# junghoseong/aircombat-selfplay

Hardware: AMD Instinct MI355X
Metric: agent-steps/sec (higher is better)
Workload: dtype f32

## Files before the change

aircombat-selfplay_amd/csrc/aircombat.hip:

```cpp
#include <hip/hip_runtime.h>
#include <stdint.h>
#include <stdio.h>
#include <string.h>
#include <string>
#include <vector>
#include <cmath>
#include <algorithm>
#include <chrono>
#include "../../include/aircombat.h"
#include "../../include/aircombat_buffer.h"
#include "clk_stamps.hpp"
#include "f16_device.hpp"
#include "f16_split.hpp"

using f16::State;
using f16::Derived;
using f16::Tab;
using f16::clampf;

#define AC_F_FIELDS(X)                                                                                           \
  X(vx) X(vy) X(vz) X(q0) X(q1) X(q2) X(q3) X(wp) X(wq) X(wr) X(hv1x) X(hv1y) X(hv1z) X(hv2x) X(hv2y) X(hv2z)   \
  X(ha1x) X(ha1y) X(ha1z) X(wdx) X(wdy) X(wdz) X(aix) X(aiy) X(aiz) X(bax) X(bay) X(baz) X(da) X(de) X(dr)       \
  X(thr) X(pin_r) X(pin_p) X(pin_y) X(pi_r) X(pi_p) X(pi_y) X(tef) X(ail) X(elev) X(sbdeg) X(alpha) X(mach)      \
  X(qc) X(vg) X(ap) X(aq) X(ar) X(npx) X(npy) X(npz) X(n1) X(n2) X(n2norm) X(ff) X(tank0) X(tank1)
// ... 156 lines not shown
    s.npz = v.x; s.npx = v.y; s.eng = __float_as_int(v.z); s.ticks = __float_as_int(v.w);
  }
  if (ROLE != 1) load_position(D, N, n, s);
}
__device__ __forceinline__ void load_flight(const float* F, const int* I, const double* D, int N, int n, State& s) { load_flight_role<-1>(F, I, D, N, n, s); }
__device__ __forceinline__ void store_flight(float* F, int* I, double* D, int N, int n, const State& s) {
  (void)I;
  AC_LANE_INDEX(n);
#define G(g, a, b, c, d) AC_GRP(F, g) = make_float4(s.a, s.b, s.c, s.d);
  AC_FLIGHT_GROUPS(G)
#undef G
  AC_GRP(F, 6) = make_float4(s.npz, s.npx, __int_as_float(s.eng), __int_as_float(s.ticks));
  store_position(D, N, n, s);
}
__device__ __forceinline__ void load_task(const float* F, const int* I, int N, int n, Task& t) {
  (void)I;
  AC_LANE_INDEX(n);
  const float4 a = AC_GRP(F, SG_TASK0), b = AC_GRP(F, SG_TASK0 + 1), c = AC_GRP(F, SG_TASK0 + 2), d = AC_GRP(F, SG_TASK0 + 3);
  t.pre_posture = a.x; t.pre_altitude = a.y; t.pre_event = a.z; t.cur_step = __float_as_int(a.w);
  t.bloods = b.x; t.status = __float_as_int(b.y); t.die_flag = __float_as_int(b.z); t.pre_shoot = b.w;
  t.remaining = __float_as_int(c.x); t.pre_remaining = __float_as_int(c.y); t.shoot_action = __float_as_int(c.z); t.last_missile = __float_as_int(c.w);
  t.last_shoot_time = __float_as_int(d.x); t.lock_bits = __float_as_int(d.y); t.lock_pos = __float_as_int(d.z);
}
__device__ __forceinline__ void store_task_group0(float* F, int N, int n, const Task& t) {
  AC_LANE_INDEX(n);
  AC_GRP(F, SG_TASK0) = make_float4(t.pre_posture, t.pre_altitude, t.pre_event, __int_as_float(t.cur_step));
}
__device__ __forceinline__ void store_task_rare(float* F, int N, int n, const Task& t) {
  AC_LANE_INDEX(n);
  AC_GRP(F, SG_TASK0 + 1) = make_float4(t.bloods, __int_as_float(t.status), __int_as_float(t.die_flag), t.pre_shoot);
  AC_GRP(F, SG_TASK0 + 2) = make_float4(__int_as_float(t.remaining), __int_as_float(t.pre_remaining), __int_as_float(t.shoot_action), __int_as_float(t.last_missile));
  AC_GRP(F, SG_TASK0 + 3) = make_float4(__int_as_float(t.last_shoot_time), __int_as_float(t.lock_bits), __int_as_float(t.lock_pos), 0.0f);
}
__device__ __forceinline__ void store_task(float* F, int* I, int N, int n, const Task& t) {
  (void)I;
  store_task_group0(F, N, n, t);
  store_task_rare(F, N, n, t);
}
__device__ __forceinline__ void load_state(const float* F, const int* I, const double* D, int N, int n, State& s, Task& t) {
  load_flight(F, I, D, N, n, s);
  load_task(F, I, N, n, t);
}
__device__ __forceinline__ void store_state(float* F, int* I, double* D, int N, int n, const State& s, const Task& t) {
  store_flight(F, I, D, N, n, s);
  store_task(F, I, N, n, t);
}
// ... 51 lines not shown
  float n, e, u;
  double n64, e64, u64;
  float vn, ve, vd;
  float alt_m;
  float ub, vb, wb, vc;
  float sphi, cphi, stht, ctht;
  float m11, m12;
};
__device__ __forceinline__ float mps(float fps) { return clampf(-700.0f, fps * f16::kFt2M, 700.0f); }

__device__ __forceinline__ void make_pose(const Derived& d, const DevCfg& c, Props& p) {
  p.alt_m = clampf(-500.0f, d.h_sl_ft * f16::kFt2M, 26000.0f);
  p.vn = mps(d.vn); p.ve = mps(d.ve); p.vd = mps(d.vd);
  const double a = 6378137.0, b = 6356752.314245179;
  double sl = d.sLat64, cl = d.cLat64, so = d.sLon64, co = d.cLon64;
  double Nn = a * a * fx::rsqrt(a * a * cl * cl + b * b * sl * sl);
  double h = (double)p.alt_m;
  double x = (Nn + h) * cl * co, y = (Nn + h) * cl * so, z = (Nn * (b / a) * (b / a) + h) * sl;
  double dx = x - c.P0x, dy = y - c.P0y, dz = z - c.P0z;
  double t = c.cLon0 * dx + c.sLon0 * dy;
  p.e64 = -c.sLon0 * dx + c.cLon0 * dy; p.u64 = c.cLat0 * t + c.sLat0 * dz; p.n64 = -c.sLat0 * t + c.cLat0 * dz;
  p.e = (float)p.e64; p.u = (float)p.u64; p.n = (float)p.n64;
}
__device__ __forceinline__ void make_props(const State& s, const Derived& d, const DevCfg& c, Props& p) {
  make_pose(d, c, p);
  p.ub = mps(d.u); p.vb = mps(d.v); p.wb = mps(d.w);
  p.vc = clampf(0.0f, f16::vcas_from_impact_pressure(s.qc) * f16::kFt2M, 1400.0f);
  const float* T = d.T;
  float m13 = T[0] * d.d_eci[0] + T[1] * d.d_eci[1] + T[2] * d.d_eci[2];
  float m23 = T[3] * d.d_eci[0] + T[4] * d.d_eci[1] + T[5] * d.d_eci[2];
  float m33 = T[6] * d.d_eci[0] + T[7] * d.d_eci[1] + T[8] * d.d_eci[2];
  p.m11 = T[0] * d.n_eci[0] + T[1] * d.n_eci[1] + T[2] * d.n_eci[2];
  p.m12 = T[0] * d.e_eci[0] + T[1] * d.e_eci[1] + T[2] * d.e_eci[2];
  p.stht = clampf(-1.0f, -m13, 1.0f);
  float ct = sqrtf(fmaxf(0.0f, 1.0f - p.stht * p.stht));
  p.ctht = ct;
  float ic = (ct > 1e-12f) ? 1.0f / sqrtf(m23 * m23 + m33 * m33) : 0.0f;
  p.sphi = (ct > 1e-12f) ? m23 * ic : 0.0f;
  p.cphi = (ct > 1e-12f) ? m33 * ic : 1.0f;
}

struct Geo { float AO, TA, R, side, cAO, cTA; };
__device__ __forceinline__ float acos_fast(float x) { return f16::atan2_fast(sqrtf((1.0f - x) * (1.0f + x)), x); }
__device__ __forceinline__ float tanh_fast(float x) {
  const float t = __expf(2.0f * clampf(-10.0f, x, 10.0f));
  return (t - 1.0f) / (t + 1.0f);
}
__device__ __forceinline__ float atanh_fast(float x) { return 0.5f * __logf((1.0f + x) / (1.0f - x)); }
template <bool TWO_D>
__device__ __forceinline__ Geo ao_ta_r(float ex, float ey, float ez, float evx, float evy, float evz,
                                       float nx, float ny, float nz, float nvx, float nvy, float nvz) {
  float dx = nx - ex, dy = ny - ey, dz = nz - ez;
  float ev, nv, R, pe, pn;
  if (TWO_D) {
    ev = sqrtf(evx * evx + evy * evy); nv = sqrtf(nvx * nvx + nvy * nvy); R = sqrtf(dx * dx + dy * dy);
    pe = dx * evx + dy * evy; pn = dx * nvx + dy * nvy;
  } else {
    ev = sqrtf(evx * evx + evy * evy + evz * evz); nv = sqrtf(nvx * nvx + nvy * nvy + nvz * nvz);
    R = sqrtf(dx * dx + dy * dy + dz * dz);
    pe = dx * evx + dy * evy + dz * evz; pn = dx * nvx + dy * nvy + dz * nvz;
  }
  Geo g;
// ... 388 lines not shown
  PairLds& LP = QUAD ? LQ.P : *reinterpret_cast<PairLds*>(split_lds);
  const Tab T{lds_tab};
  const int N = c.N;
  const int l = threadIdx.x & 63;
  const int n = blockIdx.x * 64 + l;
  const bool live = n < N;
  const int nn = live ? n : (N - 2 + (n & 1));
  const int slot = nn & 1;

  State s; Task t; Derived d; Props pr;
  int pre_st[MSLOTS];
#pragma unroll
  for (int k = 0; k < MSLOTS; ++k) pre_st[k] = MSL_INACTIVE;
  const float* act = P.actions + (size_t)nn * c.act_dim;
  float4 a4;
  ActionFetch arow;
  float shoot_raw = 0.0f;
  if (SPLIT) {
    TableCopy<192> tc;
    tc.issue(P.tab);
    AC_CLKW(0, 123);
    const int role = __builtin_amdgcn_readfirstlane(threadIdx.x >> 6);
    s = State{}; t = Task{};
    if (role == 0) { load_flight_role<0>(P.F, P.I, P.D, N, nn, s); AC_CLKW(0, 124); load_task(P.F, P.I, N, nn, t); AC_CLKW(0, 125); }
    else if (role == 1) load_flight_role<1>(P.F, P.I, P.D, N, nn, s);
    else { load_flight_role<2>(P.F, P.I, P.D, N, nn, s); t.status = state_word(P.F, SW_status, N, nn); }
    __builtin_amdgcn_s_barrier();
    tc.write(lds_tab);
    a4 = make_float4(0.f, 0.f, 0.f, 0.f);
    __builtin_amdgcn_s_waitcnt(0x0F70);
    if (role == 1) arow.issue(act, c.act_dim);
    AC_CLKW(0, 120); AC_CLKW(1, 121); AC_CLKW(2, 122);
    __syncthreads();
  } else if (QUAD) {
    const int role = __builtin_amdgcn_readfirstlane(threadIdx.x >> 6);
    TableCopy<256> tc;
    tc.issue(P.tab);
    s = State{}; t = Task{};
    if (role == 0) { load_flight_role<0>(P.F, P.I, P.D, N, nn, s); t.status = state_word(P.F, SW_status, N, nn); }
    else if (role == 1) load_flight_role<1>(P.F, P.I, P.D, N, nn, s);
    else if (role == 2) { load_flight_role<2>(P.F, P.I, P.D, N, nn, s); t.status = state_word(P.F, SW_status, N, nn); }
    else {
      load_task(P.F, P.I, N, nn, t);
      s.ticks = state_word(P.F, SW_ticks, N, nn);
#pragma unroll
      for (int k = 0; k < MSLOTS; ++k) pre_st[k] = P.MI[((size_t)k * NMI + MI_status) * (size_t)N + nn];
    }
    __builtin_amdgcn_s_barrier();
    tc.write(lds_tab);
// ... 10 lines not shown
      a4 = make_float4(0.f, 0.f, 0.f, 0.f);
      s = State{}; load_task(P.F, P.I, N, nn, t);
#pragma unroll
      for (int k = 0; k < MSLOTS; ++k) pre_st[k] = P.MI[((size_t)k * NMI + MI_status) * (size_t)N + nn];
    }
    stage_tables<128>(lds_tab, P.tab);
    if (flight_role) {
      pair_flight_load(P, c, nn, fin);
      pair_flight_wave<true>(P, c, T, LP, l, n, live, fin);
      return;
    }

  } else {
    TableCopy<64> tc;
    tc.issue(P.tab);
    a4 = load_controls(act, c.act_dim);
    if (TASK == AC_TASK_SHOOT_MISSILE) shoot_raw = act[4];
    load_state(P.F, P.I, P.D, N, nn, s, t);
    tc.commit(lds_tab);
  }
  AC_CLK(1);
  const Task was = t;
  constexpr bool OBS_BY_KIN = SPLIT && TASK == AC_TASK_SINGLECOMBAT;
  if (SPLIT) {
    const int role = __builtin_amdgcn_readfirstlane(threadIdx.x >> 6);
    if (split_helper_wave(s, t, T, L, l, c.substeps, nullptr, nullptr, &arow)) {
      if (OBS_BY_KIN && role == 1) {
        using namespace mail;
        wg_sync();
        Props q;
        q.alt_m = L.M[T_PR][l]; q.ub = L.M[T_PR + 5][l];
        q.n = L.M[T_PR + 9][l]; q.e = L.M[T_PR + 10][l]; q.u = L.M[T_PR + 11][l];
        q.vn = L.M[T_PR + 12][l]; q.ve = L.M[T_PR + 13][l]; q.vd = L.M[T_PR + 14][l];
        const Enemy Eq = exchange_1v1(q);
        L.M[T_RALT][l] = altitude_raw(q, c);
        L.M[T_RPOS][l] = posture_raw(q, Eq);
        wg_sync();
      }
      if (OBS_BY_KIN && role == 2) {
        using namespace mail;
        wg_sync();
        Props q;
        q.alt_m = L.M[T_PR][l]; q.sphi = L.M[T_PR + 1][l]; q.cphi = L.M[T_PR + 2][l]; q.stht = L.M[T_PR + 3][l]; q.ctht = L.M[T_PR + 4][l];
        q.ub = L.M[T_PR + 5][l]; q.vb = L.M[T_PR + 6][l]; q.wb = L.M[T_PR + 7][l]; q.vc = L.M[T_PR + 8][l];
        q.n = L.M[T_PR + 9][l]; q.e = L.M[T_PR + 10][l]; q.u = L.M[T_PR + 11][l];
        q.vn = L.M[T_PR + 12][l]; q.ve = L.M[T_PR + 13][l]; q.vd = L.M[T_PR + 14][l];
        const Enemy Eq = exchange_1v1(q);
        const Incoming none{false, 0, 0, 0, 0, 0, 0};
        float obq[OBS];
        observe_1v1<TASK>(q, Eq, none, obq);
        wg_sync();
        if (L.M[T_DONE][l] != 0.0f) {
          const float* tobs = (const float*)(P.tF + (size_t)NSW * 2) + slot * OBS;
#pragma unroll
          for (int k = 0; k < OBS; ++k) obq[k] = tobs[k];
        }
        float* row = lds_out + l * OBS;
#pragma unroll
        for (int k = 0; k < OBS; ++k) row[k] = obq[k];
        emit_obs_rows(P, lds_out, OBS, l);
      }
      return;
    }
  }
  Msl ms[MSLOTS];
  int nslots = 0, msl_was_active = 0;
  if (HAS_MSL) {
    nslots = min(c.num_missiles[slot], MSLOTS);
#pragma unroll
    for (int k = 0; k < MSLOTS; ++k) {
      const int st = (k < nslots) ? (PAIR ? pre_st[k] : P.MI[((size_t)k * NMI + MI_status) * (size_t)N + nn]) : MSL_INACTIVE;
      if (st != MSL_INACTIVE) { load_msl(P.MF, P.MI, N, nn, k, ms[k]); msl_was_active |= 1 << k; }
      else { ms[k] = Msl{}; ms[k].status = MSL_INACTIVE; }
    }
  }

  t.cur_step += 1;
  if (!SPLIT) {
    s.da = clampf(-1.0f, a4.x / 20.0f - 1.0f, 1.0f);
    s.de = clampf(-1.0f, a4.y / 20.0f - 1.0f, 1.0f);
    s.dr = clampf(-1.0f, a4.z / 20.0f - 1.0f, 1.0f);
    s.thr = clampf(0.0f, a4.w / 58.0f + 0.4f, 0.9f);
  }
  if (TASK == AC_TASK_SHOOT_MISSILE && !PAIR) t.shoot_action = (shoot_raw != 0.0f) ? 1 : 0;

  const MslParam MP = aim9l();
  bool have_pose = false;
  int last_tick = -1;
  bool env_has_missiles = false;
  if (PAIR) {
    bool mine = false;
#pragma unroll
    for (int k = 0; k < MSLOTS; ++k) mine = mine || ms[k].status != MSL_INACTIVE;
    const int other = __shfl_xor((int)mine, 1);
    env_has_missiles = mine || (bool)other;
  }
  int quad_nrun = 0;
  const int quad_ticks0 = s.ticks;
  for (int sub = 0; sub < c.substeps; ++sub) {
    bool fly_munitions = HAS_MSL;
    if (QUAD) {
      quad_substep_begin<true>(t, LQ, l, sub, env_has_missiles, quad_ticks0, quad_nrun, pr, c);
      fly_munitions = env_has_missiles;
    } else if (PAIR) {
      AC_CLK(2 + 8 * sub);
      pair_substep<true>(t, LP, l, sub, env_has_missiles, pr, c);
      AC_CLK(4 + 8 * sub);
      if (!env_has_missiles) continue;
    } else if (SPLIT) {
      if (dynamics_wave_tick(s, t, d, T, L, l, sub)) { have_pose = true; last_tick = sub; }
    } else if (t.status == AC_ALIVE) {
      if (t.bloods <= 0.0f) t.status = AC_SHOTDOWN;
      f16::tick<false>(s, d, T);
      have_pose = true;
    }
    if (HAS_MSL && fly_munitions) {
      if (!PAIR) {
      f16::locate(s, d);
      if (!have_pose) { f16::body_frame(s, d); have_pose = true; }
      make_props(s, d, c, pr);
      }
      float tx = __shfl_xor(pr.n, 1), ty = __shfl_xor(pr.e, 1), tz = __shfl_xor(pr.u, 1);
      float tvx = __shfl_xor(pr.vn, 1), tvy = __shfl_xor(pr.ve, 1), tvz = __shfl_xor(pr.vd, 1);
      bool talive = __shfl_xor(t.status, 1) == AC_ALIVE;
      bool hit_now = false;
#pragma unroll
      for (int k = 0; k < MSLOTS; ++k) {
        if (k < nslots && ms[k].status != MSL_INACTIVE) {
          missile_run(ms[k], MP, tx, ty, tz, tvx, tvy, tvz, talive, c);
          if (ms[k].status == MSL_HIT && talive) { hit_now = true; talive = false; }
        }
      }
      if (__shfl_xor((int)hit_now, 1) && t.status == AC_ALIVE) t.status = AC_SHOTDOWN;
      AC_CLK(5 + 8 * sub);
    }
    if (QUAD) wg_sync();
  }
  const bool split_located = SPLIT && dynamics_wave_finish(s, d, L, l, last_tick, c.substeps);
  if (PAIR) {
    if (QUAD) wg_sync();
    wg_sync();
    pair_read_final(LP, l, s, d, pr);
  } else if (!HAS_MSL || c.substeps == 0) {
    if (!split_located) f16::locate(s, d);
    if (!have_pose) f16::body_frame(s, d);
    make_props(s, d, c, pr);
  }
  AC_CLK(52);
  if (OBS_BY_KIN) {
    using namespace mail;
    L.M[T_PR][l] = pr.alt_m; L.M[T_PR + 1][l] = pr.sphi; L.M[T_PR + 2][l] = pr.cphi; L.M[T_PR + 3][l] = pr.stht; L.M[T_PR + 4][l] = pr.ctht;
    L.M[T_PR + 5][l] = pr.ub; L.M[T_PR + 6][l] = pr.vb; L.M[T_PR + 7][l] = pr.wb; L.M[T_PR + 8][l] = pr.vc;
    L.M[T_PR + 9][l] = pr.n; L.M[T_PR + 10][l] = pr.e; L.M[T_PR + 11][l] = pr.u;
    L.M[T_PR + 12][l] = pr.vn; L.M[T_PR + 13][l] = pr.ve; L.M[T_PR + 14][l] = pr.vd;
    wg_sync();
  }
  Enemy E = exchange_1v1(pr);

  if (c.use_artillery) {
    Geo g = ao_ta_r<false>(pr.n, pr.e, pr.u, pr.vn, pr.ve, pr.vd, E.n, E.e, E.u, E.vn, E.ve, E.vd);
    bool ealive = __shfl_xor(t.status, 1) == AC_ALIVE;
    float of = (g.AO <= 0.5236f) ? 1.0f - g.AO / 0.5236f : 0.0f;
    float Rk = g.R * 0.001f;
    float df = (Rk <= 1.0f) ? 1.0f : ((Rk <= 3.0f) ? (3.0f - Rk) * 0.5f : 0.0f);
    float dmg = ealive ? of * df : 0.0f;
    t.bloods -= __shfl_xor(dmg, 1);
  }
  if (HAS_MSL) {
    bool launch;
    if (TASK == AC_TASK_SHOOT_MISSILE && PAIR) t.shoot_action = ((QUAD ? LQ.S.M[mail::F_BITS][l] : LP.FIN[pair::FIN_BITS][l]) != 0.0f) ? 1 : 0;
    if (TASK == AC_TASK_DODGE_MISSILE) {
      const float dx = E.n - pr.n, dy = E.e - pr.e, dz = E.u - pr.u;
      const float dist = sqrtf(dx * dx + dy * dy + dz * dz);
      const float sp = sqrtf(pr.vn * pr.vn + pr.ve * pr.ve + pr.vd * pr.vd);
      const float ang = 57.29577951f * acosf(clampf(-1.0f, (dx * pr.vn + dy * pr.ve + dz * pr.vd) / (dist * sp + 1e-8f), 1.0f));
      const int len = c.lock_len;
      const unsigned bit = 1u << (unsigned)(t.lock_pos % len);
      t.lock_bits = (ang < c.max_attack_angle) ? (t.lock_bits | (int)bit) : (t.lock_bits & ~(int)bit);
      t.lock_pos += 1;
// ... 24 lines not shown
      t.remaining -= 1;
    }
  }

  Incoming inc{false, 0, 0, 0, 0, 0, 0};
  int my_hits = 0;
  int inc_slot = -1;
  if (HAS_MSL) {
    int best = 0x7fffffff, mine = -1;
#pragma unroll
    for (int k = 0; k < MSLOTS; ++k) {
      if (k < nslots && ms[k].status == MSL_LAUNCHED && ms[k].order < best) { best = ms[k].order; mine = k; }
      if (k < nslots && ms[k].status == MSL_HIT) my_hits += 1;
    }
    float a0 = 0, a1 = 0, a2 = 0, a3 = 0, a4 = 0, a5 = 0;
#pragma unroll
    for (int k = 0; k < MSLOTS; ++k)
      if (k == mine) { a0 = ms[k].px; a1 = ms[k].py; a2 = ms[k].pz; a3 = ms[k].vx; a4 = ms[k].vy; a5 = ms[k].vz; }
    inc.any = __shfl_xor((int)(mine >= 0), 1);
    inc_slot = __shfl_xor(mine, 1);
    inc.px = __shfl_xor(a0, 1); inc.py = __shfl_xor(a1, 1); inc.pz = __shfl_xor(a2, 1);
    inc.vx = __shfl_xor(a3, 1); inc.vy = __shfl_xor(a4, 1); inc.vz = __shfl_xor(a5, 1);
  }
  float ob[OBS];
  if (!OBS_BY_KIN) observe_1v1<TASK>(pr, E, inc, ob);
  AC_CLK(58);

  const int status_pre = t.status;
  int code = AC_DONE_NONE;
  bool done = false;
  bool nonfinite = false;
  {
    float np_max = fmaxf(fabsf(s.npx), fmaxf(fabsf(s.npy), fabsf(s.npz)));
    float pqr = sqrtf(d.p * d.p + d.q * d.q + d.r * d.r);
    nonfinite = nonfinite_probe(d.veci, pqr, d.h_sl_ft, np_max);
    bool extreme = nonfinite || (d.veci >= 1e10f) || (pqr >= 1000.0f) || (d.h_sl_ft >= 1e10f) || (np_max > 10.0f);
    bool overload = (s.ticks >= kTickOverload) &&
                    (fabsf(s.npx) > c.acc_x || fabsf(s.npy) > c.acc_y || fabsf(s.npz + 1.0f) > c.acc_z);
    if (pr.alt_m <= c.altitude_limit) { t.status = AC_CRASH; code = AC_DONE_LOW_ALTITUDE; done = true; }
    else if (extreme) { t.status = AC_CRASH; code = AC_DONE_EXTREME_STATE; done = true; }
    else if (overload) { t.status = AC_CRASH; code = AC_DONE_OVERLOAD; done = true; }
  }
  {
    int other_pre = __shfl_xor(status_pre, 1), other_post = __shfl_xor(t.status, 1);
    int enemy_status = (slot == 0) ? other_pre : other_post;
    if (!done) {
      if (t.status == AC_SHOTDOWN) { code = AC_DONE_SHOTDOWN; done = true; }
      else if (t.status == AC_CRASH) { code = AC_DONE_CRASHED; done = true; }
      else if (enemy_status != AC_ALIVE && !inc.any) { code = AC_DONE_MISSION_COMPLETE; done = true; }
      else if (t.cur_step >= c.max_steps) { code = AC_DONE_TIMEOUT; done = true; }
    }
  }

  const int other_done = __shfl_xor((int)done, 1);
  const bool all_done = done && (bool)other_done;
  const int other_code = __shfl_xor(code, 1);
  if (OBS_BY_KIN) {
    L.M[mail::T_DONE][l] = all_done ? 1.0f : 0.0f;
    wg_sync();
  } else if (all_done) {
    const float* tobs = (const float*)(P.tF + (size_t)NSW * 2) + slot * OBS;
#pragma unroll
    for (int k = 0; k < OBS; ++k) ob[k] = tobs[k];
  }

  AC_CLK(59);
  float reward = 0.0f;
  const bool evaluates = !t.die_flag;
  if (evaluates) {
    t.die_flag = (t.status != AC_ALIVE) ? 1 : 0;
    float r_alt = potential(OBS_BY_KIN ? L.M[mail::T_RALT][l] : altitude_raw(pr, c), c.altitude_scale, c.altitude_pot, t.pre_altitude);
    float r_pos = potential(OBS_BY_KIN ? L.M[mail::T_RPOS][l] : posture_raw(pr, E), c.posture_scale, c.posture_pot, t.pre_posture);
    float ev = ((t.status != AC_ALIVE) ? -200.0f : 0.0f) + 200.0f * (float)my_hits;
    float r_ev = potential(ev, c.event_scale, c.event_pot, t.pre_event);
    reward = r_alt + r_pos + r_ev;
    if (TASK == AC_TASK_SHOOT_MISSILE) {
      float sp = (t.remaining == t.pre_remaining - 1) ? -30.0f : 0.0f;
      t.pre_remaining = t.remaining;
      reward += potential(sp, c.shoot_penalty_scale, c.shoot_pot, t.pre_shoot);
    }
  }
  if (TASK == AC_TASK_DODGE_MISSILE) {
    float spd[MSLOTS];
#pragma unroll
    for (int k = 0; k < MSLOTS; ++k) spd[k] = sqrtf(ms[k].vx * ms[k].vx + ms[k].vy * ms[k].vy + ms[k].vz * ms[k].vz);
    const int base = (threadIdx.x & 63) - slot;
    const int my_inc_id = inc.any ? 1 + (slot ^ 1) * MSLOTS + inc_slot : 0;
    int prev = t.shoot_action;
    float r_mp = 0.0f;
#pragma unroll
    for (int i = 0; i < 2; ++i) {
      const int ev_i = __shfl((int)evaluates, base + i), id_i = __shfl(my_inc_id, base + i);
      if (!ev_i) continue;
      if (id_i) {
        if (!prev) prev = id_i;
        float v_prev = 0.0f, v_cur = 0.0f;
#pragma unroll
        for (int k = 0; k < MSLOTS; ++k) {
          float a = __shfl(spd[k], base + (prev - 1) / MSLOTS), b = __shfl(spd[k], base + (id_i - 1) / MSLOTS);
          if (k == (prev - 1) % MSLOTS) v_prev = a;
          if (k == (id_i - 1) % MSLOTS) v_cur = b;
        }
        if (slot == i) {
          const float v_dec = (v_prev - v_cur) / 340.0f * c.missile_posture_scale;
          const float va = sqrtf(pr.vn * pr.vn + pr.ve * pr.ve + pr.vd * pr.vd);
          const float ang = (inc.vx * pr.vn + inc.vy * pr.ve + inc.vz * pr.vd) / (v_cur * va);
          r_mp = (ang < 0.0f) ? ang / (fmaxf(v_dec, 0.0f) + 1.0f) : ang * fmaxf(v_dec, 0.0f);
        }
      } else prev = 0;
    }
    t.shoot_action = prev;
    reward += r_mp;
  }

  int step_out = t.cur_step;
  if (all_done) {
    load_state(P.tF, P.tI, P.tD, 2, slot, s, t);
    zero_controller_state(P, N, n, live);
#pragma unroll
    for (int k = 0; k < MSLOTS; ++k) { ms[k] = Msl{}; ms[k].status = MSL_INACTIVE; }
  }
  AC_CLK(53);
  if (live) {
    if (!PAIR) { store_flight(P.F, P.I, P.D, N, n, s); store_task_changed(P.F, P.I, N, n, t, was); }
    else {
      if (all_done) store_flight(P.F, P.I, P.D, N, n, s);
      store_task_changed(P.F, P.I, N, n, t, was);
    }
    if (HAS_MSL) {
#pragma unroll
      for (int k = 0; k < MSLOTS; ++k)
        if (k < nslots && (ms[k].status != MSL_INACTIVE || ((msl_was_active >> k) & 1))) store_msl(P.MF, P.MI, N, n, k, ms[k]);
    }
  }
  AC_CLK(55);
  reward = poison_if(nonfinite, reward);
  if (OBS_BY_KIN) emit_scalars(P, l, reward, done, 2, step_out, other_code ? other_code : code, 0, all_done ? 1 : 0);
  else emit_outputs(P, lds_out, OBS, l, ob, reward, done, 2, step_out, other_code ? other_code : code, 0, all_done ? 1 : 0);
  AC_CLK(54);
}

__device__ __forceinline__ Enemy gather_pose(const Props& pr, int lane) {
  Enemy E;
  E.n = __shfl(pr.n, lane); E.e = __shfl(pr.e, lane); E.u = __shfl(pr.u, lane);
  E.vn = __shfl(pr.vn, lane); E.ve = __shfl(pr.ve, lane); E.vd = __shfl(pr.vd, lane);
  E.ub = __shfl(pr.ub, lane); E.alt = __shfl(pr.alt_m, lane);
  return E;
}
template <int A>
__device__ __forceinline__ float observe_nvn(const Props& pr, int slot, int base_lane, int n_ego, float* ob) {
  auto c10 = [](float v) { return clampf(-10.0f, v, 10.0f); };
  if (ob) {
    ob[0] = c10(pr.alt_m / 5000.0f);
    ob[1] = c10(pr.sphi); ob[2] = c10(pr.cphi); ob[3] = c10(pr.stht); ob[4] = c10(pr.ctht);
    ob[5] = c10(pr.ub / 340.0f); ob[6] = c10(pr.vb / 340.0f); ob[7] = c10(pr.wb / 340.0f); ob[8] = c10(pr.vc / 340.0f);
  }
  const int my_team = slot < n_ego ? 0 : 1;
  const int n_mine = my_team == 0 ? n_ego : A - n_ego;
  float posture = 0.0f;
#pragma unroll
  for (int j = 0; j < A; ++j) {
// ... 1382 lines not shown
```

aircombat-selfplay_amd/csrc/split_kernel.hpp:

```cpp
#pragma once

namespace mail {
enum { RUNF,
       CTH, VB,
       MACH, QBAR, RHO, TEMP, HSL, ALPHA, BETA, QC, VG, NPY, NPZ, AP, AQ, AR,
       S_AIL, S_FLAP, S_ELEV, S_RUD, S_LEF, S_SB,
       THRUST,
       LK_CLB, LK_CNB, LK_G7,
       MASS0 = LK_G7 + 4, MASS_N = 18,
       F_TEF = MASS0 + MASS_N, F_PINR, F_PINP, F_PINY, F_PIR, F_PIP, F_PIY, F_AIL, F_ELEV, F_SBDEG, F_N1, F_N2, F_N2NORM, F_FF, F_TANK0, F_TANK1,
       F_ENG, F_DA, F_DE, F_DR, F_THR,
       F_BITS,
       K_W, K_V = K_W + 3,
       K_OUT = K_V + 3, K_OUT_N = 27,
       G_Q = K_OUT + K_OUT_N,
       G_H = G_Q + 8, G_NED = G_H + 1,
       QP_F = G_NED + 8, QP_F_N = 9,
       T_PR = QP_F + 2 * QP_F_N, T_PR_N = 15,
       T_DONE = T_PR + T_PR_N,
       T_RALT = T_DONE + 1, T_RPOS,
       ROWS = T_RPOS + 1 };
enum { GD_R, GD_X = GD_R + 6, GD_LAT = GD_X + 3, GD_QP = GD_LAT + 4, DROWS = GD_QP + 6 };
}
__device__ __forceinline__ void post_kin(float (*M)[64], int l, const f16::KinOut& o) {
  const float v[mail::K_OUT_N] = {o.T[0], o.T[1], o.T[2], o.T[3], o.T[4], o.T[5], o.T[6], o.T[7], o.T[8], o.h_sl_ft, o.n_eci[0], o.n_eci[1], o.n_eci[2],
                                  o.e_eci[0], o.e_eci[1], o.d_eci[0], o.d_eci[1], o.d_eci[2], o.gx, o.gy, o.gz, o.rxf, o.ryf, o.A.T, o.A.P, o.A.rho, o.A.a};
#pragma unroll
  for (int i = 0; i < mail::K_OUT_N; ++i) M[mail::K_OUT + i][l] = v[i];
}
__device__ __forceinline__ void fetch_kin(float (*M)[64], int l, f16::KinOut& o) {
  float v[mail::K_OUT_N];
#pragma unroll
  for (int i = 0; i < mail::K_OUT_N; ++i) v[i] = M[mail::K_OUT + i][l];
#pragma unroll
  for (int i = 0; i < 9; ++i) o.T[i] = v[i];
  o.h_sl_ft = v[9]; o.n_eci[0] = v[10]; o.n_eci[1] = v[11]; o.n_eci[2] = v[12]; o.e_eci[0] = v[13]; o.e_eci[1] = v[14];
  o.d_eci[0] = v[15]; o.d_eci[1] = v[16]; o.d_eci[2] = v[17]; o.gx = v[18]; o.gy = v[19]; o.gz = v[20]; o.rxf = v[21]; o.ryf = v[22];
  o.A.T = v[23]; o.A.P = v[24]; o.A.rho = v[25]; o.A.a = v[26];
}
__device__ __forceinline__ void post_mass(float (*M)[64], int l, const f16::DynVars& k) {
  const float v[mail::MASS_N] = {k.mass, k.cgx, k.cgy, k.cgz, k.Jxx, k.Jyy, k.Jzz, k.Jxy, k.Jxz, k.Jyz, k.c00, k.c01, k.c02, k.c11, k.c12, k.c22, k.idet, k.im_};
#pragma unroll
  for (int i = 0; i < mail::MASS_N; ++i) M[mail::MASS0 + i][l] = v[i];
}
// ... 152 lines not shown
      MD[GD_LAT][l] = d.sLat64; MD[GD_LAT + 1][l] = d.cLat64; MD[GD_LAT + 2][l] = d.sLon64; MD[GD_LAT + 3][l] = d.cLon64;
    }
    AC_CLKW(2, 69 + sub * 8);
    wg_sync();
    if (run) {
      f16::DynVars kl{};
      f16::Derived dd{};
      dd.h_sl_ft = 1e6f;
      kl.alpha = M[ALPHA][l]; kl.beta = M[BETA][l]; kl.mach = M[MACH][l]; kl.vt = 1.0f;
      f16::dyn_p3(dd, T, kl, f16::Surf{});
      M[LK_CLB][l] = kl.clb; M[LK_CNB][l] = kl.cnb;
      M[LK_G7][l] = kl.g7.x; M[LK_G7 + 1][l] = kl.g7.y; M[LK_G7 + 2][l] = kl.g7.z; M[LK_G7 + 3][l] = kl.g7.w;
    }
    if (run && !last) {
      f16::kin_attitude(s, o);
      post_kin(M, l, o);
    }
    AC_CLKW(2, 70 + sub * 8);
    wg_sync();
    if (POSE && run && !last) post_quad_pose(M, MD, l, (sub + 1) & 1, s, ticks0 + sub + 2, *cfg);
  }
  wg_sync();
}
struct SplitLds {
  float M[mail::ROWS][64];
  double MD[mail::DROWS][64];
};
template <bool QUAD = false, bool POSE = false>
__device__ __forceinline__ bool split_helper_wave(f16::State& s, Task& t, const f16::Tab& T, SplitLds& L, int l, int substeps, const float4* raw = nullptr,
                                                  const DevCfg* cfg = nullptr, ActionFetch* row = nullptr) {
  const int role = __builtin_amdgcn_readfirstlane(threadIdx.x >> 6);
  if (role == 2) { kinematics_wave<QUAD, POSE>(s, t, T, L.M, L.MD, l, substeps, cfg); return true; }
  if (role == 1) { systems_wave(s, t, T, L.M, l, substeps, raw, row); return true; }
  return false;
}
template <bool QUAD = false>
__device__ __forceinline__ bool dynamics_wave_tick(f16::State& s, Task& t, f16::Derived& d, const f16::Tab& T, SplitLds& L, int l, int sub, bool* d_stale = nullptr) {
  using namespace mail;
  float (*M)[64] = L.M;
  double (*MD)[64] = L.MD;
  bool run = t.status == AC_ALIVE;
  if (!QUAD && run && t.bloods <= 0.0f) t.status = AC_SHOTDOWN;
  f16::DynVars k;
  AC_CLK(2 + sub * 8);
  if (!QUAD) M[RUNF][l] = run ? 1.0f : 0.0f;
  const float b_wp = s.wp, b_wq = s.wq, b_wr = s.wr, b_vx = s.vx, b_vy = s.vy, b_vz = s.vz, b_ax = s.ha1x, b_ay = s.ha1y, b_az = s.ha1z;
  const float b_h1x = s.hv1x, b_h1y = s.hv1y, b_h1z = s.hv1z, b_h2x = s.hv2x, b_h2y = s.hv2y, b_h2z = s.hv2z;
  const int b_ticks = s.ticks;
  if (QUAD && !run) { M[K_V][l] = s.vx; M[K_V + 1][l] = s.vy; M[K_V + 2][l] = s.vz; }
  if (run) {
    if (sub == 0) f16::dyn_p1(s, d, k);
    else {
      f16::KinOut o;
      fetch_kin(M, l, o);
      f16::dyn_p1_lite(s, d, k, o);
    }
    M[K_W][l] = s.wp; M[K_W + 1][l] = s.wq; M[K_W + 2][l] = s.wr;
    M[K_V][l] = s.vx; M[K_V + 1][l] = s.vy; M[K_V + 2][l] = s.vz;
    M[CTH][l] = d.T[6] * d.d_eci[0] + d.T[7] * d.d_eci[1] + d.T[8] * d.d_eci[2];
    M[VB][l] = d.v;
  }
  AC_CLK(3 + sub * 8);
  wg_sync();
  AC_CLK(4 + sub * 8);
  if (QUAD && run && M[RUNF][l] == 0.0f) {
    s.wp = b_wp; s.wq = b_wq; s.wr = b_wr; s.vx = b_vx; s.vy = b_vy; s.vz = b_vz; s.ha1x = b_ax; s.ha1y = b_ay; s.ha1z = b_az; s.ticks = b_ticks;
    s.hv1x = b_h1x; s.hv1y = b_h1y; s.hv1z = b_h1z; s.hv2x = b_h2x; s.hv2y = b_h2y; s.hv2z = b_h2z;
    t.status = AC_SHOTDOWN;
    run = false;
    if (d_stale) *d_stale = true;
  }
  if (run) {
    fetch_mass(M, l, k);
    if (sub == 0) f16::dyn_p2<false>(s, d, k);
    else f16::dyn_p2<true>(s, d, k);
    M[BETA][l] = k.beta;
    M[MACH][l] = k.mach; M[QBAR][l] = k.qbar; M[RHO][l] = k.A.rho; M[TEMP][l] = k.A.T; M[HSL][l] = d.h_sl_ft;
    M[ALPHA][l] = k.alpha; M[QC][l] = k.qc; M[VG][l] = k.vg; M[NPY][l] = k.npy; M[NPZ][l] = k.npz;
    M[AP][l] = d.p; M[AQ][l] = d.q; M[AR][l] = d.r;
  }
  AC_CLK(5 + sub * 8);
  wg_sync();
  AC_CLK(6 + sub * 8);
  f16::Surf sf{};
  if (run) {
    sf = f16::Surf{M[S_AIL][l], M[S_FLAP][l], M[S_ELEV][l], M[S_RUD][l], M[S_LEF][l], M[S_SB][l], 0.0f};
    f16::dyn_p3(d, T, k, sf);
  }
  AC_CLK(7 + sub * 8);
  wg_sync();
  AC_CLK(8 + sub * 8);
  if (run) {
    k.clb = M[LK_CLB][l]; k.cnb = M[LK_CNB][l];
    k.g7 = make_float4(M[LK_G7][l], M[LK_G7 + 1][l], M[LK_G7 + 2][l], M[LK_G7 + 3][l]);
    f16::dyn_p4(s, d, k, sf, M[THRUST][l]);
    if (sub > 0) {
      const int pb = sub & 1;
      s.rx = MD[GD_R + 3 * pb][l]; s.ry = MD[GD_R + 3 * pb + 1][l]; s.rz = MD[GD_R + 3 * pb + 2][l];
    }
  }
  return run;
}
__device__ __forceinline__ bool dynamics_wave_finish(f16::State& s, f16::Derived& d, SplitLds& L, int l, int last_tick, int substeps) {
  using namespace mail;
  float (*M)[64] = L.M;
  double (*MD)[64] = L.MD;
  AC_CLK(50);
  wg_sync();
  AC_CLK(51);
  s.tef = M[F_TEF][l]; s.pin_r = M[F_PINR][l]; s.pin_p = M[F_PINP][l]; s.pin_y = M[F_PINY][l];
  s.pi_r = M[F_PIR][l]; s.pi_p = M[F_PIP][l]; s.pi_y = M[F_PIY][l]; s.ail = M[F_AIL][l]; s.elev = M[F_ELEV][l]; s.sbdeg = M[F_SBDEG][l];
  s.n1 = M[F_N1][l]; s.n2 = M[F_N2][l]; s.n2norm = M[F_N2NORM][l]; s.ff = M[F_FF][l]; s.tank0 = M[F_TANK0][l]; s.tank1 = M[F_TANK1][l];
  s.eng = __float_as_int(M[F_ENG][l]);
  s.da = M[F_DA][l]; s.de = M[F_DE][l]; s.dr = M[F_DR][l]; s.thr = M[F_THR][l];
  if (last_tick >= 1) {
    const int pb = last_tick & 1;
    s.q0 = M[G_Q + 4 * pb][l]; s.q1 = M[G_Q + 4 * pb + 1][l]; s.q2 = M[G_Q + 4 * pb + 2][l]; s.q3 = M[G_Q + 4 * pb + 3][l];
  }
  if (last_tick < 0 || last_tick != substeps - 1) return false;
  d.X = MD[GD_X][l]; d.Y = MD[GD_X + 1][l]; d.Z = MD[GD_X + 2][l];
  d.sLat64 = MD[GD_LAT][l]; d.cLat64 = MD[GD_LAT + 1][l]; d.sLon64 = MD[GD_LAT + 2][l]; d.cLon64 = MD[GD_LAT + 3][l];
  d.h_sl_ft = M[G_H][l];
  d.n_eci[0] = M[G_NED][l]; d.n_eci[1] = M[G_NED + 1][l]; d.n_eci[2] = M[G_NED + 2][l];
  d.e_eci[0] = M[G_NED + 3][l]; d.e_eci[1] = M[G_NED + 4][l]; d.e_eci[2] = 0.0f;
  d.d_eci[0] = M[G_NED + 5][l]; d.d_eci[1] = M[G_NED + 6][l]; d.d_eci[2] = M[G_NED + 7][l];
  return true;
}
__device__ __forceinline__ bool dynamics_wave_ticks(f16::State& s, Task& t, f16::Derived& d, const f16::Tab& T, SplitLds& L, int l, int substeps,
                                                    int& nrun) {
  int last_tick = -1;
  nrun = 0;
  for (int sub = 0; sub < substeps; ++sub)
    if (dynamics_wave_tick(s, t, d, T, L, l, sub)) { last_tick = sub; nrun += 1; }
  const bool located = dynamics_wave_finish(s, d, L, l, last_tick, substeps);
  if (last_tick >= 0 && !located) { f16::locate(s, d); return true; }
  return located;
}
```

Measured before the change: 234.0 million.

## Move env/reward/obs work onto kinematics wave in split kernel

Restructures the three-wave SingleCombat kernel: the kinematics wave now runs the environment step itself (locate, pose, observation, reward, task stores), the dynamics wave only flies and stores flight state, and the systems wave only emits observation rows. Before, pose props were staged through LDS and observation/reward raw values were computed redundantly on helper waves with extra barriers. Dynamics now publishes body-frame data to new mailbox rows on the last tick, so kinematics can build props without recomputing. This rebalances work across waves and removes the LDS prop round-trip, at the cost of more complex cross-wave synchronisation and a higher chance of ordering bugs.

```diff
diff --git a/aircombat-selfplay_amd/csrc/aircombat.hip b/aircombat-selfplay_amd/csrc/aircombat.hip
--- a/aircombat-selfplay_amd/csrc/aircombat.hip
+++ b/aircombat-selfplay_amd/csrc/aircombat.hip
@@ -202,6 +202,11 @@
   t.remaining = __float_as_int(c.x); t.pre_remaining = __float_as_int(c.y); t.shoot_action = __float_as_int(c.z); t.last_missile = __float_as_int(c.w);
   t.last_shoot_time = __float_as_int(d.x); t.lock_bits = __float_as_int(d.y); t.lock_pos = __float_as_int(d.z);
 }
+__device__ __forceinline__ void load_task_status(const float* F, int N, int n, Task& t) {
+  AC_LANE_INDEX(n);
+  const float4 b = AC_GRP(F, SG_TASK0 + 1);
+  t.bloods = b.x; t.status = __float_as_int(b.y);
+}
 __device__ __forceinline__ void store_task_group0(float* F, int N, int n, const Task& t) {
   AC_LANE_INDEX(n);
   AC_GRP(F, SG_TASK0) = make_float4(t.pre_posture, t.pre_altitude, t.pre_event, __int_as_float(t.cur_step));
@@ -299,8 +304,7 @@
   p.e64 = -c.sLon0 * dx + c.cLon0 * dy; p.u64 = c.cLat0 * t + c.sLat0 * dz; p.n64 = -c.sLat0 * t + c.cLat0 * dz;
   p.e = (float)p.e64; p.u = (float)p.u64; p.n = (float)p.n64;
 }
-__device__ __forceinline__ void make_props(const State& s, const Derived& d, const DevCfg& c, Props& p) {
-  make_pose(d, c, p);
+__device__ __forceinline__ void make_body_props(const State& s, const Derived& d, Props& p) {
   p.ub = mps(d.u); p.vb = mps(d.v); p.wb = mps(d.w);
   p.vc = clampf(0.0f, f16::vcas_from_impact_pressure(s.qc) * f16::kFt2M, 1400.0f);
   const float* T = d.T;
@@ -315,6 +319,10 @@
   float ic = (ct > 1e-12f) ? 1.0f / sqrtf(m23 * m23 + m33 * m33) : 0.0f;
   p.sphi = (ct > 1e-12f) ? m23 * ic : 0.0f;
   p.cphi = (ct > 1e-12f) ? m33 * ic : 1.0f;
+}
+__device__ __forceinline__ void make_props(const State& s, const Derived& d, const DevCfg& c, Props& p) {
+  make_pose(d, c, p);
+  make_body_props(s, d, p);
 }
 
 struct Geo { float AO, TA, R, side, cAO, cTA; };
@@ -749,9 +757,12 @@
     AC_CLKW(0, 123);
     const int role = __builtin_amdgcn_readfirstlane(threadIdx.x >> 6);
     s = State{}; t = Task{};
-    if (role == 0) { load_flight_role<0>(P.F, P.I, P.D, N, nn, s); AC_CLKW(0, 124); load_task(P.F, P.I, N, nn, t); AC_CLKW(0, 125); }
+    if (role == 0) { load_flight_role<0>(P.F, P.I, P.D, N, nn, s); AC_CLKW(0, 124); load_task_status(P.F, N, nn, t); AC_CLKW(0, 125); }
     else if (role == 1) load_flight_role<1>(P.F, P.I, P.D, N, nn, s);
-    else { load_flight_role<2>(P.F, P.I, P.D, N, nn, s); t.status = state_word(P.F, SW_status, N, nn); }
+    else {
+      load_flight_role<2>(P.F, P.I, P.D, N, nn, s); load_task(P.F, P.I, N, nn, t);
+      s.qc = __int_as_float(state_word(P.F, SW_qc, N, nn)); s.npy = __int_as_float(state_word(P.F, SW_npy, N, nn));
+    }
     __builtin_amdgcn_s_barrier();
     tc.write(lds_tab);
     a4 = make_float4(0.f, 0.f, 0.f, 0.f);
@@ -808,46 +819,44 @@
   AC_CLK(1);
   const Task was = t;
   constexpr bool OBS_BY_KIN = SPLIT && TASK == AC_TASK_SINGLECOMBAT;
+  static_assert(OBS_BY_KIN == SPLIT, "the three-wave form of this kernel is SingleCombat's");
   if (SPLIT) {
+    using namespace mail;
     const int role = __builtin_amdgcn_readfirstlane(threadIdx.x >> 6);
-    if (split_helper_wave(s, t, T, L, l, c.substeps, nullptr, nullptr, &arow)) {
-      if (OBS_BY_KIN && role == 1) {
-        using namespace mail;
-        wg_sync();
-        Props q;
-        q.alt_m = L.M[T_PR][l]; q.ub = L.M[T_PR + 5][l];
-        q.n = L.M[T_PR + 9][l]; q.e = L.M[T_PR + 10][l]; q.u = L.M[T_PR + 11][l];
-        q.vn = L.M[T_PR + 12][l]; q.ve = L.M[T_PR + 13][l]; q.vd = L.M[T_PR + 14][l];
-        const Enemy Eq = exchange_1v1(q);
-        L.M[T_RALT][l] = altitude_raw(q, c);
-        L.M[T_RPOS][l] = posture_raw(q, Eq);
-        wg_sync();
+    if (role == 1) {
+      systems_wave(s, t, T, L.M, l, c.substeps, nullptr, &arow);
+      AC_CLKW(1, 203);
+      emit_obs_rows(P, lds_out, OBS, l);
+      AC_CLKW(1, 206);
+      return;
+    }
+    if (role == 0) {
+      int last_tick = -1;
+      for (int sub = 0; sub < c.substeps; ++sub)
+        if (dynamics_wave_tick<false, true>(s, t, d, T, L, l, sub, nullptr, sub + 1 == c.substeps)) last_tick = sub;
+      dynamics_wave_finish<false>(s, d, L, l, last_tick, c.substeps);
+      AC_CLK(53);
+      if (L.M[T_DONE][l] != 0.0f) {
+        load_flight(P.tF, P.tI, P.tD, 2, slot, s);
+        zero_controller_state(P, N, n, live);
       }
-      if (OBS_BY_KIN && role == 2) {
-        using namespace mail;
-        wg_sync();
-        Props q;
-        q.alt_m = L.M[T_PR][l]; q.sphi = L.M[T_PR + 1][l]; q.cphi = L.M[T_PR + 2][l]; q.stht = L.M[T_PR + 3][l]; q.ctht = L.M[T_PR + 4][l];
-        q.ub = L.M[T_PR + 5][l]; q.vb = L.M[T_PR + 6][l]; q.wb = L.M[T_PR + 7][l]; q.vc = L.M[T_PR + 8][l];
-        q.n = L.M[T_PR + 9][l]; q.e = L.M[T_PR + 10][l]; q.u = L.M[T_PR + 11][l];
-        q.vn = L.M[T_PR + 12][l]; q.ve = L.M[T_PR + 13][l]; q.vd = L.M[T_PR + 14][l];
-        const Enemy Eq = exchange_1v1(q);
-        const Incoming none{false, 0, 0, 0, 0, 0, 0};
-        float obq[OBS];
-        observe_1v1<TASK>(q, Eq, none, obq);
-        wg_sync();
-        if (L.M[T_DONE][l] != 0.0f) {
-          const float* tobs = (const float*)(P.tF + (size_t)NSW * 2) + slot * OBS;
-#pragma unroll
-          for (int k = 0; k < OBS; ++k) obq[k] = tobs[k];
-        }
-        float* row = lds_out + l * OBS;
-#pragma unroll
-        for (int k = 0; k < OBS; ++k) row[k] = obq[k];
-        emit_obs_rows(P, lds_out, OBS, l);
-      }
+      if (live) store_flight(P.F, P.I, P.D, N, n, s);
+      AC_CLK(55);
       return;
     }
+    const int lt = kinematics_wave_env(s, t, T, L.M, L.MD, l, c.substeps, c, d, pr);
+    AC_CLKW(2, 200);
+    if (lt >= 0) {
+#pragma unroll
+      for (int i = 0; i < E_T_N; ++i) d.T[i] = L.M[E_T + i][l];
+      d.u = L.M[E_U][l]; d.v = L.M[VB][l]; d.w = L.M[E_W][l];
+      d.p = L.M[AP][l]; d.q = L.M[AQ][l]; d.r = L.M[AR][l];
+      d.vn = L.M[E_VN][l]; d.ve = L.M[E_VE][l]; d.vd = L.M[E_VD][l]; d.veci = L.M[E_VECI][l];
+      s.qc = L.M[QC][l]; s.npx = L.M[E_NPX][l]; s.npy = L.M[NPY][l]; s.npz = L.M[NPZ][l];
+      t.status = __float_as_int(L.M[E_STATUS][l]);
+    } else f16::body_frame(s, d);
+    pr.vn = mps(d.vn); pr.ve = mps(d.ve); pr.vd = mps(d.vd);
+    make_body_props(s, d, pr);
   }
   Msl ms[MSLOTS];
   int nslots = 0, msl_was_active = 0;
@@ -872,7 +881,6 @@
 
   const MslParam MP = aim9l();
   bool have_pose = false;
-  int last_tick = -1;
   bool env_has_missiles = false;
   if (PAIR) {
     bool mine = false;
@@ -883,7 +891,7 @@
   }
   int quad_nrun = 0;
   const int quad_ticks0 = s.ticks;
-  for (int sub = 0; sub < c.substeps; ++sub) {
+  for (int sub = 0; !SPLIT && sub < c.substeps; ++sub) {
     bool fly_munitions = HAS_MSL;
     if (QUAD) {
       quad_substep_begin<true>(t, LQ, l, sub, env_has_missiles, quad_ticks0, quad_nrun, pr, c);
@@ -893,8 +901,6 @@
       pair_substep<true>(t, LP, l, sub, env_has_missiles, pr, c);
       AC_CLK(4 + 8 * sub);
       if (!env_has_missiles) continue;
-    } else if (SPLIT) {
-      if (dynamics_wave_tick(s, t, d, T, L, l, sub)) { have_pose = true; last_tick = sub; }
     } else if (t.status == AC_ALIVE) {
       if (t.bloods <= 0.0f) t.status = AC_SHOTDOWN;
       f16::tick<false>(s, d, T);
@@ -922,25 +928,16 @@
     }
     if (QUAD) wg_sync();
   }
-  const bool split_located = SPLIT && dynamics_wave_finish(s, d, L, l, last_tick, c.substeps);
   if (PAIR) {
     if (QUAD) wg_sync();
     wg_sync();
     pair_read_final(LP, l, s, d, pr);
-  } else if (!HAS_MSL || c.substeps == 0) {
-    if (!split_located) f16::locate(s, d);
+  } else if (!SPLIT && (!HAS_MSL || c.substeps == 0)) {
+    f16::locate(s, d);
     if (!have_pose) f16::body_frame(s, d);
     make_props(s, d, c, pr);
   }
   AC_CLK(52);
-  if (OBS_BY_KIN) {
-    using namespace mail;
-    L.M[T_PR][l] = pr.alt_m; L.M[T_PR + 1][l] = pr.sphi; L.M[T_PR + 2][l] = pr.cphi; L.M[T_PR + 3][l] = pr.stht; L.M[T_PR + 4][l] = pr.ctht;
-    L.M[T_PR + 5][l] = pr.ub; L.M[T_PR + 6][l] = pr.vb; L.M[T_PR + 7][l] = pr.wb; L.M[T_PR + 8][l] = pr.vc;
-    L.M[T_PR + 9][l] = pr.n; L.M[T_PR + 10][l] = pr.e; L.M[T_PR + 11][l] = pr.u;
-    L.M[T_PR + 12][l] = pr.vn; L.M[T_PR + 13][l] = pr.ve; L.M[T_PR + 14][l] = pr.vd;
-    wg_sync();
-  }
   Enemy E = exchange_1v1(pr);
 
   if (c.use_artillery) {
@@ -1011,8 +1008,10 @@
     inc.px = __shfl_xor(a0, 1); inc.py = __shfl_xor(a1, 1); inc.pz = __shfl_xor(a2, 1);
     inc.vx = __shfl_xor(a3, 1); inc.vy = __shfl_xor(a4, 1); inc.vz = __shfl_xor(a5, 1);
   }
+  AC_CLKW(2, 201);
+  if (SPLIT && c.substeps > 0) wg_sync();
   float ob[OBS];
-  if (!OBS_BY_KIN) observe_1v1<TASK>(pr, E, inc, ob);
+  observe_1v1<TASK>(pr, E, inc, ob);
   AC_CLK(58);
 
   const int status_pre = t.status;
@@ -1044,22 +1043,27 @@
   const int other_done = __shfl_xor((int)done, 1);
   const bool all_done = done && (bool)other_done;
   const int other_code = __shfl_xor(code, 1);
-  if (OBS_BY_KIN) {
+  if (all_done) {
+    const float* tobs = (const float*)(P.tF + (size_t)NSW * 2) + slot * OBS;
+#pragma unroll
+    for (int k = 0; k < OBS; ++k) ob[k] = tobs[k];
+  }
+  if (SPLIT) {
+    float* row = lds_out + l * OBS;
+#pragma unroll
+    for (int k = 0; k < OBS; ++k) row[k] = ob[k];
     L.M[mail::T_DONE][l] = all_done ? 1.0f : 0.0f;
+    AC_CLKW(2, 202);
     wg_sync();
-  } else if (all_done) {
-    const float* tobs = (const float*)(P.tF + (size_t)NSW * 2) + slot * OBS;
-#pragma unroll
-    for (int k = 0; k < OBS; ++k) ob[k] = tobs[k];
-  }
-
-  AC_CLK(59);
+  }
+
+  AC_CLK(59); AC_CLKW(2, 204);
   float reward = 0.0f;
   const bool evaluates = !t.die_flag;
   if (evaluates) {
     t.die_flag = (t.status != AC_ALIVE) ? 1 : 0;
-    float r_alt = potential(OBS_BY_KIN ? L.M[mail::T_RALT][l] : altitude_raw(pr, c), c.altitude_scale, c.altitude_pot, t.pre_altitude);
-    float r_pos = potential(OBS_BY_KIN ? L.M[mail::T_RPOS][l] : posture_raw(pr, E), c.posture_scale, c.posture_pot, t.pre_posture);
+    float r_alt = potential(altitude_raw(pr, c), c.altitude_scale, c.altitude_pot, t.pre_altitude);
+    float r_pos = potential(posture_raw(pr, E), c.posture_scale, c.posture_pot, t.pre_posture);
     float ev = ((t.status != AC_ALIVE) ? -200.0f : 0.0f) + 200.0f * (float)my_hits;
     float r_ev = potential(ev, c.event_scale, c.event_pot, t.pre_event);
     reward = r_alt + r_pos + r_ev;
@@ -1103,13 +1107,21 @@
   }
 
   int step_out = t.cur_step;
-  if (all_done) {
+  if (all_done && SPLIT) load_task(P.tF, P.tI, 2, slot, t);
+  else if (all_done) {
     load_state(P.tF, P.tI, P.tD, 2, slot, s, t);
     zero_controller_state(P, N, n, live);
 #pragma unroll
     for (int k = 0; k < MSLOTS; ++k) { ms[k] = Msl{}; ms[k].status = MSL_INACTIVE; }
   }
   AC_CLK(53);
+  reward = poison_if(nonfinite, reward);
+  if (SPLIT) {
+    emit_scalars(P, l, reward, done, 2, step_out, other_code ? other_code : code, 0, all_done ? 1 : 0);
+    if (live) store_task_changed(P.F, P.I, N, n, t, was);
+    AC_CLKW(2, 205);
+    return;
+  }
   if (live) {
     if (!PAIR) { store_flight(P.F, P.I, P.D, N, n, s); store_task_changed(P.F, P.I, N, n, t, was); }
     else {
@@ -1123,9 +1135,7 @@
     }
   }
   AC_CLK(55);
-  reward = poison_if(nonfinite, reward);
-  if (OBS_BY_KIN) emit_scalars(P, l, reward, done, 2, step_out, other_code ? other_code : code, 0, all_done ? 1 : 0);
-  else emit_outputs(P, lds_out, OBS, l, ob, reward, done, 2, step_out, other_code ? other_code : code, 0, all_done ? 1 : 0);
+  emit_outputs(P, lds_out, OBS, l, ob, reward, done, 2, step_out, other_code ? other_code : code, 0, all_done ? 1 : 0);
   AC_CLK(54);
 }
 
diff --git a/aircombat-selfplay_amd/csrc/split_kernel.hpp b/aircombat-selfplay_amd/csrc/split_kernel.hpp
--- a/aircombat-selfplay_amd/csrc/split_kernel.hpp
+++ b/aircombat-selfplay_amd/csrc/split_kernel.hpp
@@ -16,10 +16,11 @@
        G_Q = K_OUT + K_OUT_N,
        G_H = G_Q + 8, G_NED = G_H + 1,
        QP_F = G_NED + 8, QP_F_N = 9,
-       T_PR = QP_F + 2 * QP_F_N, T_PR_N = 15,
-       T_DONE = T_PR + T_PR_N,
-       T_RALT = T_DONE + 1, T_RPOS,
-       ROWS = T_RPOS + 1 };
+       E_T = QP_F + 2 * QP_F_N, E_T_N = 9,
+       E_U = E_T + E_T_N, E_W, E_VN, E_VE, E_VD, E_VECI, E_NPX,
+       E_STATUS,
+       T_DONE,
+       ROWS = T_DONE + 1 };
 enum { GD_R, GD_X = GD_R + 6, GD_LAT = GD_X + 3, GD_QP = GD_LAT + 4, DROWS = GD_QP + 6 };
 }
 __device__ __forceinline__ void post_kin(float (*M)[64], int l, const f16::KinOut& o) {
@@ -218,6 +219,71 @@
   }
   wg_sync();
 }
+__device__ __forceinline__ void kin_env_locate(double rx, double ry, double rz, int ticks, f16::Derived& d) {
+  f16::State sp{};
+  sp.rx = rx; sp.ry = ry; sp.rz = rz; sp.ticks = ticks;
+  f16::locate(sp, d);
+}
+__device__ __forceinline__ int kinematics_wave_env(f16::State& s, const Task& t, const f16::Tab& T, float (*M)[64], double (*MD)[64], int l, int substeps,
+                                                   const DevCfg& c, f16::Derived& d, Props& pr) {
+  using namespace mail;
+  f16::KinOut o;
+  const int ticks0 = s.ticks;
+  const bool alive0 = t.status == AC_ALIVE && substeps > 0;
+  if (alive0) { f16::kin_position(s, o); f16::kin_attitude(s, o); }
+  int lt = -1;
+  if (substeps == 0) {
+    kin_env_locate(s.rx, s.ry, s.rz, ticks0, d);
+    d.vn = 0.0f; d.ve = 0.0f; d.vd = 0.0f;
+    make_pose(d, c, pr);
+  }
+  for (int sub = 0; sub < substeps; ++sub) {
+    const bool last = sub + 1 == substeps;
+    if (last) kin_env_locate(s.rx, s.ry, s.rz, ticks0 + (alive0 ? substeps : 0), d);
+    AC_CLKW(2, 68 + sub * 8);
+    wg_sync();
+    const bool run = M[RUNF][l] != 0.0f;
+    if (run) {
+      const int pb = sub & 1;
+      lt = sub;
+      MD[GD_R + 3 * pb][l] = s.rx; MD[GD_R + 3 * pb + 1][l] = s.ry; MD[GD_R + 3 * pb + 2][l] = s.rz;
+      M[G_Q + 4 * pb][l] = s.q0; M[G_Q + 4 * pb + 1][l] = s.q1; M[G_Q + 4 * pb + 2][l] = s.q2; M[G_Q + 4 * pb + 3][l] = s.q3;
+    }
+    if (run && !last) {
+      s.wp = M[K_W][l]; s.wq = M[K_W + 1][l]; s.wr = M[K_W + 2][l];
+      s.vx = M[K_V][l]; s.vy = M[K_V + 1][l]; s.vz = M[K_V + 2][l];
+      f16::kin_position(s, o);
+    }
+    if (last) {
+      if (alive0 && !run) {
+        const int pb = lt & 1;
+        kin_env_locate(MD[GD_R + 3 * pb][l], MD[GD_R + 3 * pb + 1][l], MD[GD_R + 3 * pb + 2][l], ticks0 + lt + 1, d);
+      }
+      s.ticks = ticks0 + lt + 1;
+      d.vn = 0.0f; d.ve = 0.0f; d.vd = 0.0f;
+      make_pose(d, c, pr);
+    }
+    AC_CLKW(2, 69 + sub * 8);
+    wg_sync();
+    if (run) {
+      f16::DynVars kl{};
+      f16::Derived dd{};
+      dd.h_sl_ft = 1e6f;
+      kl.alpha = M[ALPHA][l]; kl.beta = M[BETA][l]; kl.mach = M[MACH][l]; kl.vt = 1.0f;
+      f16::dyn_p3(dd, T, kl, f16::Surf{});
+      M[LK_CLB][l] = kl.clb; M[LK_CNB][l] = kl.cnb;
+      M[LK_G7][l] = kl.g7.x; M[LK_G7 + 1][l] = kl.g7.y; M[LK_G7 + 2][l] = kl.g7.z; M[LK_G7 + 3][l] = kl.g7.w;
+    }
+    if (last) break;
+    if (run) {
+      f16::kin_attitude(s, o);
+      post_kin(M, l, o);
+    }
+    AC_CLKW(2, 70 + sub * 8);
+    wg_sync();
+  }
+  return lt;
+}
 struct SplitLds {
   float M[mail::ROWS][64];
   double MD[mail::DROWS][64];
@@ -230,8 +296,9 @@
   if (role == 1) { systems_wave(s, t, T, L.M, l, substeps, raw, row); return true; }
   return false;
 }
-template <bool QUAD = false>
-__device__ __forceinline__ bool dynamics_wave_tick(f16::State& s, Task& t, f16::Derived& d, const f16::Tab& T, SplitLds& L, int l, int sub, bool* d_stale = nullptr) {
+template <bool QUAD = false, bool ENVK = false>
+__device__ __forceinline__ bool dynamics_wave_tick(f16::State& s, Task& t, f16::Derived& d, const f16::Tab& T, SplitLds& L, int l, int sub, bool* d_stale = nullptr,
+                                                   bool last = false) {
   using namespace mail;
   float (*M)[64] = L.M;
   double (*MD)[64] = L.MD;
@@ -274,6 +341,12 @@
     M[MACH][l] = k.mach; M[QBAR][l] = k.qbar; M[RHO][l] = k.A.rho; M[TEMP][l] = k.A.T; M[HSL][l] = d.h_sl_ft;
     M[ALPHA][l] = k.alpha; M[QC][l] = k.qc; M[VG][l] = k.vg; M[NPY][l] = k.npy; M[NPZ][l] = k.npz;
     M[AP][l] = d.p; M[AQ][l] = d.q; M[AR][l] = d.r;
+    if (ENVK && (last || t.status != AC_ALIVE)) {
+#pragma unroll
+      for (int i = 0; i < E_T_N; ++i) M[E_T + i][l] = d.T[i];
+      M[E_U][l] = d.u; M[E_W][l] = d.w; M[E_VN][l] = d.vn; M[E_VE][l] = d.ve; M[E_VD][l] = d.vd; M[E_VECI][l] = d.veci;
+      M[E_NPX][l] = k.npx; M[E_STATUS][l] = __int_as_float(t.status);
+    }
   }
   AC_CLK(5 + sub * 8);
   wg_sync();
@@ -297,6 +370,7 @@
   }
   return run;
 }
+template <bool LOCATED = true>
 __device__ __forceinline__ bool dynamics_wave_finish(f16::State& s, f16::Derived& d, SplitLds& L, int l, int last_tick, int substeps) {
   using namespace mail;
   float (*M)[64] = L.M;
@@ -313,7 +387,7 @@
     const int pb = last_tick & 1;
     s.q0 = M[G_Q + 4 * pb][l]; s.q1 = M[G_Q + 4 * pb + 1][l]; s.q2 = M[G_Q + 4 * pb + 2][l]; s.q3 = M[G_Q + 4 * pb + 3][l];
   }
-  if (last_tick < 0 || last_tick != substeps - 1) return false;
+  if (!LOCATED || last_tick < 0 || last_tick != substeps - 1) return false;
   d.X = MD[GD_X][l]; d.Y = MD[GD_X + 1][l]; d.Z = MD[GD_X + 2][l];
   d.sLat64 = MD[GD_LAT][l]; d.cLat64 = MD[GD_LAT + 1][l]; d.sLon64 = MD[GD_LAT + 2][l]; d.cLon64 = MD[GD_LAT + 3][l];
   d.h_sl_ft = M[G_H][l];
```

Result: no change. 236.4 million, median of 3 (+1.0%).
